# dsshim0125/s2p

Hardware: AMD Instinct MI355X
Metric: G+D train-step images/sec at 84x84 bs=64/GPU (higher is better)
Workload: dtype bf16; 1 GPU; configs[2]: full G+D train step (hinge GAN + feature matching + VGG19 perceptual + L1, Adam x2), 84x84 cheetah, netG=s2p, netD=multiscale(2); global_batch=64, per_gpu_batch=64, parallelism=dp1, hip_graph=True, graph_segments=1, streams=overlapped, vgg_weights=seeded stand-in (ImageNet weights unobtainable offline)

## Files before the change

s2p_amd/csrc/wgrad_head.hip:

```cpp
#include "s2p_common.h"

struct HeadArgs {
  const __bf16* x; const __bf16* dy; float* dw; float* db; float* part;
  int N, H, W, Cin, x_pitch, Ho, Wo, y_pitch, KH, KW, pad;
  int cin_real, nchunk, rpb, npix, iters, G;
  int wpi;
};

template <int KH_, int KW_>
__global__ __launch_bounds__(256) void head_wgrad_kernel(const HeadArgs a) {
  constexpr int MAXT = KH_ > 0 ? KH_ * KW_ : 16;
  __shared__ float red[256 * 8];
  const int KW = KW_ > 0 ? KW_ : a.KW;
  const int T = KH_ > 0 ? KH_ * KW_ : a.KH * a.KW;
  const int ch = threadIdx.x % a.nchunk, row = threadIdx.x / a.nchunk;
  float acc[MAXT][8];
#pragma unroll
  for (int t = 0; t < MAXT; ++t)
#pragma unroll
    for (int e = 0; e < 8; ++e) acc[t][e] = 0.f;
  const int HW = a.H * a.W;
  for (int it = 0; it < a.iters; ++it) {
    const int pi = (it * a.G + blockIdx.x) * a.rpb + row;
    if (pi >= a.npix || row >= a.rpb) continue;
    const int n = pi / HW, rr = pi - n * HW, iy = rr / a.W, ix = rr - iy * a.W;
    Chunk<__bf16> xv;
    xv.raw = *(const u32x4*)(a.x + (size_t)pi * a.x_pitch + ch * 8);
    const __bf16* dyn = a.dy + (size_t)n * a.Ho * a.Wo * a.y_pitch;
    float d[MAXT];
#pragma unroll
    for (int t = 0; t < MAXT; ++t) {
      const int ky = t / KW, kx = t - ky * KW;
      const int oy = iy + a.pad - ky, ox = ix + a.pad - kx;
      const bool ok = t < T && oy >= 0 && oy < a.Ho && ox >= 0 && ox < a.Wo;
      const int oyc = oy < 0 ? 0 : (oy >= a.Ho ? a.Ho - 1 : oy), oxc = ox < 0 ? 0 : (ox >= a.Wo ? a.Wo - 1 : ox);
      const float v = (float)dyn[(size_t)(oyc * a.Wo + oxc) * a.y_pitch];
      d[t] = ok ? v : 0.f;
    }
    float xf[8];
#pragma unroll
    for (int e = 0; e < 8; ++e) xf[e] = xv.get(e);
#pragma unroll
    for (int t = 0; t < MAXT; ++t)
#pragma unroll
      for (int e = 0; e < 8; ++e) acc[t][e] = __builtin_fmaf(d[t], xf[e], acc[t][e]);
  }
  float* part = a.part + (size_t)blockIdx.x * T * a.Cin;
#pragma unroll
  for (int t = 0; t < MAXT; ++t) {
    if (t < T) {
      __syncthreads();
      if (row < a.rpb) {
#pragma unroll
        for (int e = 0; e < 8; ++e) red[(row * a.nchunk + ch) * 8 + e] = acc[t][e];
      }
      __syncthreads();
      for (int c = threadIdx.x; c < a.Cin; c += 256) {
        float s = 0.f;
        for (int r = 0; r < a.rpb; ++r) s += red[r * a.Cin + c];
        part[t * a.Cin + c] = s;
      }
    }
  }
}

template <int R>
__global__ __launch_bounds__(256, 2) void head_wgrad_stream_kernel(const HeadArgs a) {
  constexpr int T = 16, KW = 4;
  __shared__ __attribute__((aligned(1024))) char ring[4 * R * 1024];
  __shared__ float hmap[400];
  const int tid = threadIdx.x, lane = tid & 63;
  const int wave = __builtin_amdgcn_readfirstlane(tid >> 6);
  const int n = blockIdx.x / a.wpi, part_i = blockIdx.x - n * a.wpi;
  const int HW = a.H * a.W, nmap = a.Ho * a.Wo;
  const int per = (HW + a.wpi - 1) / a.wpi, p0 = part_i * per, p1 = p0 + per < HW ? p0 + per : HW;
  for (int i = tid; i < nmap; i += 256) hmap[i] = (float)a.dy[((size_t)n * nmap + i) * a.y_pitch];
  __syncthreads();
  const i32x4 rs = s2p_make_rsrc(a.x + (size_t)n * HW * a.x_pitch, (unsigned)HW * (unsigned)a.x_pitch * 2u);
  const unsigned ring_lds = __builtin_amdgcn_readfirstlane(s2p_lds_addr(ring)) + (unsigned)wave * (R * 1024);
  const int npx = p1 - p0 - wave > 0 ? (p1 - p0 - wave + 3) >> 2 : 0;
  auto issue = [&](int i) {
    const int p = p0 + wave + 4 * i;
    s2p_dma16(rs, ring_lds + (unsigned)((i % R) * 1024), i < npx ? p * a.x_pitch * 2 + lane * 16 : (int)0x80000000);
  };
#pragma unroll
  for (int i = 0; i < R; ++i) issue(i);
  float acc[T][8];
#pragma unroll
  for (int t = 0; t < T; ++t)
#pragma unroll
    for (int e = 0; e < 8; ++e) acc[t][e] = 0.f;
  for (int i = 0; i < npx; ++i) {
    S2P_WAIT_VMCNT(R - 1);
    Chunk<__bf16> xv;
    xv.raw = *(const u32x4*)(ring + (wave * R + (i % R)) * 1024 + lane * 16);
    asm volatile("s_waitcnt lgkmcnt(0)" ::: "memory");
    issue(i + R);
    const int p = p0 + wave + 4 * i, iy = p / a.W, ix = p - iy * a.W;
    float d[T];
#pragma unroll
    for (int t = 0; t < T; ++t) {
      const int ky = t / KW, kx = t - ky * KW;
      const int oy = iy + a.pad - ky, ox = ix + a.pad - kx;
      const bool ok = oy >= 0 && oy < a.Ho && ox >= 0 && ox < a.Wo;
      d[t] = ok ? hmap[oy * a.Wo + ox] : 0.f;
    }
    float xf[8];
#pragma unroll
    for (int e = 0; e < 8; ++e) xf[e] = xv.get(e);
#pragma unroll
    for (int t = 0; t < T; ++t)
#pragma unroll
      for (int e = 0; e < 8; ++e) acc[t][e] = __builtin_fmaf(d[t], xf[e], acc[t][e]);
  }
  S2P_WAIT_VMCNT(0);
  __syncthreads();
  float* red = (float*)ring;
  float* part = a.part + (size_t)blockIdx.x * T * a.Cin;
#pragma unroll
  for (int t = 0; t < T; ++t) {
    if (t) __syncthreads();
#pragma unroll
    for (int e = 0; e < 8; ++e) red[wave * 512 + lane * 8 + e] = acc[t][e];
    __syncthreads();
    for (int c = tid; c < 512; c += 256) part[t * a.Cin + c] = ((red[c] + red[512 + c]) + red[1024 + c]) + red[1536 + c];
  }
}

__global__ __launch_bounds__(1024) void head_wgrad_reduce_kernel(const HeadArgs a) {
  const int T = a.KH * a.KW;
  constexpr int NSEG = 16;
  __shared__ float red[1024];
  if (blockIdx.x < gridDim.x - 1) {
    const int o = threadIdx.x & 63, sg = threadIdx.x >> 6;
    const int i = blockIdx.x * 64 + o;
    const int per = (a.G + NSEG - 1) / NSEG;
    const int g0 = sg * per, g1 = g0 + per < a.G ? g0 + per : a.G;
    float s = 0.f;
    if (i < T * a.Cin) {
      const float* p = a.part + i;
      const size_t st = (size_t)T * a.Cin;
      int g = g0;
      for (; g + 8 <= g1; g += 8) {
        float v[8];
#pragma unroll
        for (int u = 0; u < 8; ++u) v[u] = p[(size_t)(g + u) * st];
#pragma unroll
        for (int u = 0; u < 8; ++u) s += v[u];
      }
      for (; g < g1; ++g) s += p[(size_t)g * st];
    }
    red[threadIdx.x] = s;
    __syncthreads();
    if (sg == 0 && i < T * a.Cin) {
      const int t = i / a.Cin, c = i - t * a.Cin;
      float tot = 0.f;
#pragma unroll
      for (int k = 0; k < NSEG; ++k) tot += red[64 * k + o];
      if (c < a.cin_real) a.dw[t * a.cin_real + c] += tot;
    }
    return;
  }
  if (!a.db) return;
  const long long cnt = (long long)a.N * a.Ho * a.Wo;
  float s = 0.f;
  for (long long p = threadIdx.x; p < cnt; p += 1024) s += (float)a.dy[(size_t)p * a.y_pitch];
  red[threadIdx.x] = s;
  __syncthreads();
  if (threadIdx.x == 0) {
    float t = 0.f;
    for (int k = 0; k < 1024; ++k) t += red[k];
    a.db[0] += t;
  }
}

bool s2p_head_wgrad_supported(const s2p_conv_desc* d, int cin_real, int cout_real) {
  if (d->dtype != S2P_BF16 || d->transposed || d->reflect || d->groups != 1 || d->stride != 1) return false;
  if (d->Cout != 1 || cout_real != 1 || d->KH * d->KW > 16) return false;
  const int nchunk = d->Cin / 8;
  if (d->Cin % 8 || nchunk < 1 || nchunk > 256 || 256 % nchunk) return false;
  if (cin_real > d->Cin) return false;
  return true;
}

static int head_stream_wpi(const s2p_conv_desc* d) {
  if (S2P_DIAG_SWITCH(12) || d->Cin != 512 || d->KH != 4 || d->KW != 4 || d->Ho * d->Wo > 400 || d->x_pitch % 8) return 0;
  if ((long long)d->H * d->W * d->x_pitch * 2 >= (1ll << 31)) return 0;
  int wpi = (512 + d->N - 1) / d->N;
  const int HW = d->H * d->W;
  if (wpi > (HW + 7) / 8) wpi = (HW + 7) / 8;
  return wpi < 1 ? 1 : wpi;
}

static int head_groups(const s2p_conv_desc* d) {
  if (const int wpi = head_stream_wpi(d)) return d->N * wpi;
  const int rpb = 256 / (d->Cin / 8);
  const long long npix = (long long)d->N * d->H * d->W;
  long long g = (npix + (long long)rpb * 8 - 1) / ((long long)rpb * 8);
  if (g > 512) g = 512;
  if (g < 1) g = 1;
  return (int)g;
}

size_t s2p_head_wgrad_workspace(const s2p_conv_desc* d) {
  return (size_t)head_groups(d) * d->KH * d->KW * d->Cin * sizeof(float);
}

int s2p_head_wgrad(const s2p_conv_desc* d, const void* x, const void* dy, float* dw, float* db, int cin_real,
                   void* workspace, size_t workspace_bytes, hipStream_t st) {
  HeadArgs a{};
  a.x = (const __bf16*)x; a.dy = (const __bf16*)dy; a.dw = dw; a.db = db; a.part = (float*)workspace;
  a.N = d->N; a.H = d->H; a.W = d->W; a.Cin = d->Cin; a.x_pitch = d->x_pitch; a.Ho = d->Ho; a.Wo = d->Wo;
  a.y_pitch = d->y_pitch; a.KH = d->KH; a.KW = d->KW; a.pad = d->pad; a.cin_real = cin_real;
  a.nchunk = d->Cin / 8; a.rpb = 256 / a.nchunk; a.npix = d->N * d->H * d->W;
  a.G = head_groups(d);
  a.iters = cdiv(a.npix, (long long)a.G * a.rpb);
  if (!workspace || workspace_bytes < s2p_head_wgrad_workspace(d)) S2P_FAIL(-1, "s2p_head_wgrad: workspace too small");
  a.wpi = head_stream_wpi(d);
  if (a.wpi) hipLaunchKernelGGL((head_wgrad_stream_kernel<16>), dim3(a.G), dim3(256), 0, st, a);
  else if (a.KH == 4 && a.KW == 4) hipLaunchKernelGGL((head_wgrad_kernel<4, 4>), dim3(a.G), dim3(256), 0, st, a);
  else hipLaunchKernelGGL((head_wgrad_kernel<0, 0>), dim3(a.G), dim3(256), 0, st, a);
  S2P_CHECK_LAUNCH("head_wgrad_kernel");
  const int T = a.KH * a.KW;
  hipLaunchKernelGGL(head_wgrad_reduce_kernel, dim3(cdiv(T * a.Cin, 64) + 1), dim3(1024), 0, st, a);
  S2P_CHECK_LAUNCH("head_wgrad_reduce_kernel");
  return 0;
}

struct HeadFwdArgs {
  const __bf16* x; const __bf16* w; const float* bias; __bf16* y;
  int N, H, W, x_pitch, Ho, Wo, y_pitch, pad, act;
  float slope;
};

__global__ __launch_bounds__(1024) void head_fwd_kernel(const HeadFwdArgs a) {
  constexpr int KS = 4, T = 16, MAXW = 24;
  __shared__ float patch[16][KS][MAXW];
  const int tid = threadIdx.x, lane = tid & 63;
  const int iy = __builtin_amdgcn_readfirstlane(tid >> 6);
  const int n = blockIdx.x;
  for (int i = tid; i < 16 * KS * MAXW; i += blockDim.x) (&patch[0][0][0])[i] = 0.f;
  u32x4 wv[T];
#pragma unroll
  for (int t = 0; t < T; ++t) wv[t] = *(const u32x4*)(a.w + (size_t)t * 512 + lane * 8);
  __syncthreads();
  const __bf16* xrow = a.x + ((size_t)(n * a.H + iy) * a.W) * a.x_pitch + lane * 8;
  const int kyl = (lane & 15) >> 2, kxl = lane & 3;
  u32x4 xv = *(const u32x4*)xrow;
  for (int ix = 0; ix < a.W; ++ix) {
    const u32x4 cur = xv;
    if (ix + 1 < a.W) xv = *(const u32x4*)(xrow + (size_t)(ix + 1) * a.x_pitch);
    float d[T];
#pragma unroll
    for (int t = 0; t < T; ++t) {
      float s = 0.f;
#pragma unroll
      for (int i = 0; i < 4; ++i)
        s = __builtin_amdgcn_fdot2_f32_bf16(__builtin_bit_cast(__attribute__((ext_vector_type(2))) __bf16, (unsigned)cur[i]),
                                            __builtin_bit_cast(__attribute__((ext_vector_type(2))) __bf16, (unsigned)wv[t][i]), s, false);
      d[t] = s;
    }
#define S2P_BFLY(B)                                                                         \
    {                                                                                        \
      const bool up = (lane >> (B)) & 1;                                                     \
      _Pragma("unroll") for (int i = 0; i < (1 << (B)); ++i) {                               \
        const float send = up ? d[i] : d[i + (1 << (B))];                                    \
        const float keep = up ? d[i + (1 << (B))] : d[i];                                    \
        d[i] = keep + __shfl_xor(send, 1 << (B), 64);                                        \
      }                                                                                      \
    }
    S2P_BFLY(3) S2P_BFLY(2) S2P_BFLY(1) S2P_BFLY(0)
#undef S2P_BFLY
    float v = d[0];
    v += __shfl_xor(v, 16, 64);
    v += __shfl_xor(v, 32, 64);
    if (lane < 16) {
      const int ox = ix + a.pad - kxl;
      if (ox >= 0 && ox < a.Wo) patch[iy][kyl][ox] += v;
    }
  }
  __syncthreads();
  for (int o = tid; o < a.Ho * a.Wo; o += blockDim.x) {
    const int oy = o / a.Wo, ox = o - oy * a.Wo;
    float s = a.bias ? a.bias[0] : 0.f;
#pragma unroll
    for (int ky = 0; ky < KS; ++ky) {
      const int r = oy + ky - a.pad;
      if (r >= 0 && r < a.H) s += patch[r][ky][ox];
    }
    Chunk<__bf16> c; c.raw = (u32x4){0u, 0u, 0u, 0u};
    c.set(0, act_fwd(s, a.act, a.slope));
    *(u32x4*)(a.y + ((size_t)(n * a.Ho + oy) * a.Wo + ox) * a.y_pitch) = c.raw;
  }
}

__global__ __launch_bounds__(1024) void head_fwd_mfma_kernel(const HeadFwdArgs a) {
  constexpr int KS = 4, T = 16, NS = 16;
  __shared__ float P[256][T + 1];
  const int tid = threadIdx.x, lane = tid & 63;
  const int tile = __builtin_amdgcn_readfirstlane(tid >> 6);
  const int q = lane >> 4, l15 = lane & 15;
  const int n = blockIdx.x, HW = a.H * a.W;
  int p = tile * 16 + l15;
  const bool pok = p < HW;
  if (!pok) p = HW - 1;
  const __bf16* xp = a.x + ((size_t)n * HW + p) * a.x_pitch + 8 * q;
  const __bf16* wp = a.w + (size_t)l15 * 512 + 8 * q;
  bf16x8 xa[NS], wb[NS];
#pragma unroll
  for (int s = 0; s < NS; ++s) xa[s] = *(const bf16x8*)(xp + 32 * s);
#pragma unroll
  for (int s = 0; s < NS; ++s) wb[s] = *(const bf16x8*)(wp + 32 * s);
  typedef __attribute__((ext_vector_type(4))) float f32x4h;
  f32x4h acc = {0.f, 0.f, 0.f, 0.f};
#pragma unroll
  for (int s = 0; s < NS; ++s) acc = __builtin_amdgcn_mfma_f32_16x16x32_bf16(xa[s], wb[s], acc, 0, 0, 0);
#pragma unroll
  for (int e = 0; e < 4; ++e) P[tile * 16 + 4 * q + e][l15] = acc[e];
  __syncthreads();
  for (int o = tid; o < a.Ho * a.Wo; o += blockDim.x) {
    const int oy = o / a.Wo, ox = o - oy * a.Wo;
    float sum = a.bias ? a.bias[0] : 0.f;
#pragma unroll
    for (int ky = 0; ky < KS; ++ky)
#pragma unroll
      for (int kx = 0; kx < KS; ++kx) {
        const int iy = oy - a.pad + ky, ix = ox - a.pad + kx;
        if (iy >= 0 && iy < a.H && ix >= 0 && ix < a.W) sum += P[iy * a.W + ix][ky * KS + kx];
      }
    Chunk<__bf16> c; c.raw = (u32x4){0u, 0u, 0u, 0u};
    c.set(0, act_fwd(sum, a.act, a.slope));
    *(u32x4*)(a.y + ((size_t)(n * a.Ho + oy) * a.Wo + ox) * a.y_pitch) = c.raw;
  }
}

bool s2p_head_fwd_applicable(const s2p_conv_desc* d) {
  return d->dtype == S2P_BF16 && d->groups == 1 && !d->transposed && !d->reflect && d->stride == 1 && d->Cout == 1 &&
         d->KH == 4 && d->KW == 4 && d->Cin == 512 && d->x_pitch % 8 == 0 && d->y_pitch == 8 && d->H <= 16 && d->Wo <= 24 &&
         d->H >= 1 && d->W >= 1;
}

bool s2p_head_fwd_mfma(const s2p_conv_desc* d) { return !S2P_DIAG_SWITCH(13) && d->H * d->W <= 256; }

int s2p_head_fwd(const s2p_conv_desc* d, const void* x, const void* w, const float* bias, void* y, int act, float slope,
                 bool mfma, hipStream_t st) {
  HeadFwdArgs a{};
  a.x = (const __bf16*)x; a.w = (const __bf16*)w; a.bias = bias; a.y = (__bf16*)y;
  a.N = d->N; a.H = d->H; a.W = d->W; a.x_pitch = d->x_pitch; a.Ho = d->Ho; a.Wo = d->Wo; a.y_pitch = d->y_pitch;
  a.pad = d->pad; a.act = act; a.slope = slope;
  if (mfma) {
    hipLaunchKernelGGL(head_fwd_mfma_kernel, dim3(d->N), dim3(64 * cdiv(d->H * d->W, 16)), 0, st, a);
    S2P_CHECK_LAUNCH("head_fwd_mfma_kernel");
    return 0;
  }
  hipLaunchKernelGGL(head_fwd_kernel, dim3(d->N), dim3(64 * d->H), 0, st, a);
  S2P_CHECK_LAUNCH("head_fwd_kernel");
  return 0;
}
```

Measured before the change: 8075 images/sec.

## Add MFMA-based weight-gradient kernel for Cout=1 discriminator head conv

Adds a new head weight-gradient kernel that handles one image and a channel slice per block. It DMA-loads the input tile into swizzled LDS, builds a 16-tap shifted dy matrix, and uses bf16 16x16x32 MFMA with transposed LDS reads to produce per-image partials, replacing the scalar FMA and stream kernels for small 4x4 heads. The reduce kernel also gets a 4-wide tail loop, a 4-way unrolled bias sum, and a two-level tree in place of a serial 1024-element sum. The cost is more LDS per block and a G=N partial-sum layout that the reduce kernel must walk.

```diff
diff --git a/s2p_amd/csrc/wgrad_head.hip b/s2p_amd/csrc/wgrad_head.hip
--- a/s2p_amd/csrc/wgrad_head.hip
+++ b/s2p_amd/csrc/wgrad_head.hip
@@ -5,6 +5,7 @@
   int N, H, W, Cin, x_pitch, Ho, Wo, y_pitch, KH, KW, pad;
   int cin_real, nchunk, rpb, npix, iters, G;
   int wpi;
+  int csl;
 };
 
 template <int KH_, int KW_>
@@ -148,6 +149,13 @@
 #pragma unroll
         for (int u = 0; u < 8; ++u) s += v[u];
       }
+      for (; g + 4 <= g1; g += 4) {
+        float v[4];
+#pragma unroll
+        for (int u = 0; u < 4; ++u) v[u] = p[(size_t)(g + u) * st];
+#pragma unroll
+        for (int u = 0; u < 4; ++u) s += v[u];
+      }
       for (; g < g1; ++g) s += p[(size_t)g * st];
     }
     red[threadIdx.x] = s;
@@ -164,14 +172,100 @@
   if (!a.db) return;
   const long long cnt = (long long)a.N * a.Ho * a.Wo;
   float s = 0.f;
-  for (long long p = threadIdx.x; p < cnt; p += 1024) s += (float)a.dy[(size_t)p * a.y_pitch];
+  long long p = threadIdx.x;
+  for (; p + 3 * 1024 < cnt; p += 4 * 1024) {
+    const float v0 = (float)a.dy[(size_t)p * a.y_pitch], v1 = (float)a.dy[(size_t)(p + 1024) * a.y_pitch];
+    const float v2 = (float)a.dy[(size_t)(p + 2048) * a.y_pitch], v3 = (float)a.dy[(size_t)(p + 3072) * a.y_pitch];
+    s += v0; s += v1; s += v2; s += v3;
+  }
+  for (; p < cnt; p += 1024) s += (float)a.dy[(size_t)p * a.y_pitch];
   red[threadIdx.x] = s;
   __syncthreads();
+  float t = 0.f;
+  if (threadIdx.x < 64) {
+#pragma unroll
+    for (int k = 0; k < 16; ++k) t += red[threadIdx.x * 16 + k];
+  }
+  __syncthreads();
+  if (threadIdx.x < 64) red[threadIdx.x] = t;
+  __syncthreads();
   if (threadIdx.x == 0) {
-    float t = 0.f;
-    for (int k = 0; k < 1024; ++k) t += red[k];
-    a.db[0] += t;
-  }
+    float tot = 0.f;
+    for (int k = 0; k < 64; ++k) tot += red[k];
+    a.db[0] += tot;
+  }
+}
+
+constexpr int HW_AM_RS = 264;
+__device__ __forceinline__ int head_wg_swz(int pixel) { return ((pixel & 3) | (((pixel >> 3) & 1) << 2)) << 1; }
+
+__global__ __launch_bounds__(256) void head_wgrad_mfma_kernel(const HeadArgs a) {
+  extern __shared__ __attribute__((aligned(1024))) char smem[];
+  const int tid = threadIdx.x, lane = tid & 63;
+  const int wave = __builtin_amdgcn_readfirstlane(tid >> 6);
+  const int kg = lane >> 4, l15 = lane & 15, q = (lane >> 2) & 3, p = lane & 3;
+  const int n = blockIdx.x, c_base = blockIdx.y * a.csl;
+  const int HW = a.H * a.W, nmap = a.Ho * a.Wo, ns = (HW + 31) >> 5;
+  const int rs = a.csl * 2, lpp = a.csl >> 3, lsh = a.csl == 128 ? 4 : 3;
+  char* xt = smem;
+  __bf16* Am = (__bf16*)(smem + ns * 32 * rs);
+  __bf16* map = Am + 16 * HW_AM_RS;
+  const i32x4 rsrc = s2p_make_rsrc(a.x + (size_t)n * HW * a.x_pitch, (unsigned)HW * (unsigned)a.x_pitch * 2u);
+  const unsigned xt_lds = __builtin_amdgcn_readfirstlane(s2p_lds_addr(xt));
+  const int npiece = (ns * 32 * rs) >> 10;
+  for (int i = wave; i < npiece; i += 4) {
+    const int pixel = (i << (6 - lsh)) + (lane >> lsh), c = lane & (lpp - 1);
+    const int chan = c_base + ((c ^ (head_wg_swz(pixel) & (lpp - 1))) << 3);
+    const bool ok = pixel < HW && chan < a.Cin;
+    s2p_dma16(rsrc, xt_lds + (unsigned)i * 1024u, ok ? (pixel * a.x_pitch + chan) * 2 : (int)0x80000000);
+  }
+  for (int i = tid; i < nmap; i += 256) map[i] = a.dy[((size_t)n * nmap + i) * a.y_pitch];
+  __syncthreads();
+  if (tid < ns * 32) {
+    const int iy = tid / a.W, ix = tid - iy * a.W;
+#pragma unroll
+    for (int t = 0; t < 16; ++t) {
+      const int oy = iy + a.pad - (t >> 2), ox = ix + a.pad - (t & 3);
+      const bool ok = tid < HW && oy >= 0 && oy < a.Ho && ox >= 0 && ox < a.Wo;
+      const __bf16 v = map[ok ? oy * a.Wo + ox : 0];
+      Am[t * HW_AM_RS + tid] = ok ? v : (__bf16)0.f;
+    }
+  }
+  S2P_WAIT_VMCNT(0);
+  __syncthreads();
+  const int ntile = ((a.Cin - c_base < a.csl ? a.Cin - c_base : a.csl)) >> 4;
+  typedef __attribute__((address_space(3))) s16x4* lds_s16x4;
+  f32x4 acc[2] = {{0.f, 0.f, 0.f, 0.f}, {0.f, 0.f, 0.f, 0.f}};
+  for (int s = 0; s < ns; ++s) {
+    const bf16x8 af = *(const bf16x8*)(Am + l15 * HW_AM_RS + 32 * s + 8 * kg);
+    const int pr = 32 * s + 8 * kg + q, sw = head_wg_swz(pr) & (lpp - 1);
+#pragma unroll
+    for (int i = 0; i < 2; ++i) {
+      const int cg = wave + 4 * i;
+      if (cg < ntile) {
+        const char* base = xt + pr * rs + (((2 * cg + (p >> 1)) ^ sw) << 4) + 8 * (p & 1);
+        const s16x4 lo = __builtin_amdgcn_ds_read_tr16_b64_v4i16((lds_s16x4)(base));
+        const s16x4 hi = __builtin_amdgcn_ds_read_tr16_b64_v4i16((lds_s16x4)(base + 4 * rs));
+        const bf16x8 bfr = __builtin_bit_cast(bf16x8, __builtin_shufflevector(lo, hi, 0, 1, 2, 3, 4, 5, 6, 7));
+        acc[i] = __builtin_amdgcn_mfma_f32_16x16x32_bf16(af, bfr, acc[i], 0, 0, 0);
+      }
+    }
+  }
+  float* part = a.part + (size_t)n * 16 * a.Cin + c_base;
+#pragma unroll
+  for (int i = 0; i < 2; ++i) {
+    const int cg = wave + 4 * i;
+    if (cg < ntile) {
+#pragma unroll
+      for (int e = 0; e < 4; ++e) part[(size_t)(4 * kg + e) * a.Cin + cg * 16 + l15] = acc[i][e];
+    }
+  }
+}
+
+static int head_mfma_csl(const s2p_conv_desc* d) {
+  if (S2P_DIAG_SWITCH(21) || d->KH != 4 || d->KW != 4 || d->Cin % 32 || d->H * d->W > 256 || d->Ho * d->Wo > 1024) return 0;
+  if (d->x_pitch % 8 || d->x_pitch > 65536 || d->pad < 0 || d->y_pitch < 8 || d->N < 1) return 0;
+  return (cdiv(d->H * d->W, 32) > 6 || d->Cin < 128) ? 64 : 128;
 }
 
 bool s2p_head_wgrad_supported(const s2p_conv_desc* d, int cin_real, int cout_real) {
@@ -184,6 +278,7 @@
 }
 
 static int head_stream_wpi(const s2p_conv_desc* d) {
+  if (head_mfma_csl(d)) return 0;
   if (S2P_DIAG_SWITCH(12) || d->Cin != 512 || d->KH != 4 || d->KW != 4 || d->Ho * d->Wo > 400 || d->x_pitch % 8) return 0;
   if ((long long)d->H * d->W * d->x_pitch * 2 >= (1ll << 31)) return 0;
   int wpi = (512 + d->N - 1) / d->N;
@@ -193,6 +288,7 @@
 }
 
 static int head_groups(const s2p_conv_desc* d) {
+  if (head_mfma_csl(d)) return d->N;
   if (const int wpi = head_stream_wpi(d)) return d->N * wpi;
   const int rpb = 256 / (d->Cin / 8);
   const long long npix = (long long)d->N * d->H * d->W;
@@ -217,7 +313,11 @@
   a.iters = cdiv(a.npix, (long long)a.G * a.rpb);
   if (!workspace || workspace_bytes < s2p_head_wgrad_workspace(d)) S2P_FAIL(-1, "s2p_head_wgrad: workspace too small");
   a.wpi = head_stream_wpi(d);
-  if (a.wpi) hipLaunchKernelGGL((head_wgrad_stream_kernel<16>), dim3(a.G), dim3(256), 0, st, a);
+  a.csl = head_mfma_csl(d);
+  if (a.csl) {
+    const size_t lds = (size_t)cdiv(a.H * a.W, 32) * 32 * a.csl * 2 + 16 * HW_AM_RS * 2 + 1024 * 2;
+    hipLaunchKernelGGL(head_wgrad_mfma_kernel, dim3(a.N, cdiv(a.Cin, a.csl)), dim3(256), lds, st, a);
+  } else if (a.wpi) hipLaunchKernelGGL((head_wgrad_stream_kernel<16>), dim3(a.G), dim3(256), 0, st, a);
   else if (a.KH == 4 && a.KW == 4) hipLaunchKernelGGL((head_wgrad_kernel<4, 4>), dim3(a.G), dim3(256), 0, st, a);
   else hipLaunchKernelGGL((head_wgrad_kernel<0, 0>), dim3(a.G), dim3(256), 0, st, a);
   S2P_CHECK_LAUNCH("head_wgrad_kernel");
```

Result: no change. 8110 images/sec (median of 5 runs) (+0.4%).
